# Gadersd/whisper-burn

Hardware: NVIDIA H100
Metric: audio-seconds/sec (higher is better)
Workload: dtype f32 (fp16-exact weights, fp32 activations/accumulate)

## Files before the change

### whisper-burn_b200/csrc/decoder4.cu

```cuda
#include <cooperative_groups.h>

#include "dec_common.cuh"

namespace cg = cooperative_groups;

namespace wb {

namespace {

#ifndef D4_ASYNC
#define D4_ASYNC 1
#endif
#define D4_EXCHANGE(IDX, RXBYTES, SEND, PF)                  \
    do {                                                     \
        WB_FINE();                                           \
        __syncthreads();                                     \
        WB_FINE();                                           \
        SEND();                                              \
        WB_FINE();                                           \
        if (D4_ASYNC) {                                      \
            PF();                                            \
            WB_FINE();                                       \
            xwait(xbar + (IDX), (RXBYTES), lc & 1u);         \
        } else {                                             \
            cluster_arrive();                                \
            PF();                                            \
            WB_FINE();                                       \
            cluster_wait();                                  \
        }                                                    \
    } while (0)
#ifndef D4_FINE
#define D4_FINE 0
#endif
#if D4_FINE
#define WB_FINE() WB_TRACE()
#else
#define WB_FINE() do { } while (0)
#endif

constexpr int CS = 16;
constexpr int LG_NBUF = 3;
constexpr int LG_RB = 8;
constexpr int KV_STG = 4;
#ifndef D4_L2_CKV_KEEP
#define D4_L2_CKV_KEEP 0
#endif
__device__ __forceinline__ uint64_t ckv_policy() { return D4_L2_CKV_KEEP ? l2_policy_evict_last() : l2_policy_evict_first(); }

__device__ __forceinline__ uint32_t smem_u32(const void* p) { return (uint32_t)__cvta_generic_to_shared(p); }
__device__ __forceinline__ void mbar_init(uint64_t* bar, uint32_t count) {
    asm volatile("mbarrier.init.shared::cta.b64 [%0], %1;" ::"r"(smem_u32(bar)), "r"(count));
}
__device__ __forceinline__ void mbar_expect_tx(uint64_t* bar, uint32_t bytes) {
    asm volatile("mbarrier.arrive.expect_tx.shared::cta.b64 _, [%0], %1;" ::"r"(smem_u32(bar)), "r"(bytes) : "memory");
}
__device__ __forceinline__ void mbar_wait(uint64_t* bar, uint32_t parity) {
    asm volatile(
        "{\n"
        ".reg .pred p;\n"
        "LG_WAIT:\n"
        "mbarrier.try_wait.parity.shared::cta.b64 p, [%0], %1;\n"
        "@p bra LG_DONE;\n"
        "bra LG_WAIT;\n"
        "LG_DONE:\n"
        "}\n" ::"r"(smem_u32(bar)),
        "r"(parity)
        : "memory");
}
__device__ __forceinline__ void cp_async16(void* dst, const void* src) {
    asm volatile("cp.async.cg.shared.global [%0], [%1], 16;" ::"r"(smem_u32(dst)), "l"(src) : "memory");
}
__device__ __forceinline__ void cp_async_wait_all() { asm volatile("cp.async.wait_all;" ::: "memory"); }

__device__ __forceinline__ void cluster_arrive() { asm volatile("barrier.cluster.arrive.release.aligned;" ::: "memory"); }
__device__ __forceinline__ void cluster_wait() { asm volatile("barrier.cluster.wait.acquire.aligned;" ::: "memory"); }

template <int NR, int VPL>
struct RowRegs {
    uint4 v[NR][VPL];
    float bias[NR];
    float bias_own;
};

template <int NR, int VPL>
__device__ __forceinline__ void load_rows(const __half* __restrict__ W, const float* __restrict__ bias, int K, int row0, int step,
                                          RowRegs<NR, VPL>& r, uint64_t pol) {
    const int lane = threadIdx.x & 31, nv = K / 8;
#pragma unroll
    for (int i = 0; i < NR; ++i) r.bias[i] = __ldg(bias + row0 + i * step);
    r.bias_own = __ldg(bias + row0 + min(lane >> 1, NR - 1) * step);
#pragma unroll
    for (int i = 0; i < NR; ++i) {
        const uint4* p = reinterpret_cast<const uint4*>(W + (int64_t)(row0 + i * step) * K);
#pragma unroll
        for (int j = 0; j < VPL; ++j) {
            const int v = j * 32 + lane;
            r.v[i][j] = v < nv ? ldg_l2(p + v, pol) : make_uint4(0, 0, 0, 0);
        }
    }
}
template <int NR>
__device__ __forceinline__ float warp_reduce_owner(const float (&acc)[NR]) {
    const int lane = threadIdx.x & 31;
    float v8[8], v4[4], v2[2];
    {
        const bool up = lane & 16;
#pragma unroll
        for (int i = 0; i < 8; ++i) {
            const float lo = i < NR ? acc[i] : 0.0f, hi = i + 8 < NR ? acc[i + 8] : 0.0f;
            const float recv = __shfl_xor_sync(0xffffffffu, up ? lo : hi, 16);
            v8[i] = (up ? hi : lo) + recv;
        }
    }
    {
        const bool up = lane & 8;
#pragma unroll
        for (int i = 0; i < 4; ++i) {
            const float recv = __shfl_xor_sync(0xffffffffu, up ? v8[i] : v8[i + 4], 8);
            v4[i] = (up ? v8[i + 4] : v8[i]) + recv;
        }
    }
    {
        const bool up = lane & 4;
#pragma unroll
        for (int i = 0; i < 2; ++i) {
            const float recv = __shfl_xor_sync(0xffffffffu, up ? v4[i] : v4[i + 2], 4);
            v2[i] = (up ? v4[i + 2] : v4[i]) + recv;
        }
    }
    const bool up = lane & 2;
    float v = (up ? v2[1] : v2[0]) + __shfl_xor_sync(0xffffffffu, up ? v2[0] : v2[1], 2);
    v += __shfl_xor_sync(0xffffffffu, v, 1);
    return v;
}

template <int NR, int VPL, bool REDUCE = true>
__device__ __forceinline__ void dot_rows1(const RowRegs<NR, VPL>& r, const float* xs, int K, float (&acc)[NR]) {
    const int lane = threadIdx.x & 31, nv = K / 8;
#pragma unroll
    for (int i = 0; i < NR; ++i) acc[i] = 0.0f;
#pragma unroll
    for (int j = 0; j < VPL; ++j) {
        const int v = j * 32 + lane;
        if (v < nv) {
            const float4 x0 = *reinterpret_cast<const float4*>(xs + v * 8);
            const float4 x1 = *reinterpret_cast<const float4*>(xs + v * 8 + 4);
#pragma unroll
            for (int i = 0; i < NR; ++i) {
                float w[8];
                cvt8(r.v[i][j], w);
                float a = acc[i];
                a = fmaf(w[0], x0.x, a); a = fmaf(w[1], x0.y, a); a = fmaf(w[2], x0.z, a); a = fmaf(w[3], x0.w, a);
                a = fmaf(w[4], x1.x, a); a = fmaf(w[5], x1.y, a); a = fmaf(w[6], x1.z, a); a = fmaf(w[7], x1.w, a);
                acc[i] = a;
            }
        }
    }
    if constexpr (REDUCE) {
#pragma unroll
        for (int i = 0; i < NR; ++i) acc[i] = warp_sum(acc[i]);
    }
}

__device__ __forceinline__ uint32_t mapa_u32(uint32_t addr, uint32_t rank) {
    uint32_t r;
    asm volatile("mapa.shared::cluster.u32 %0, %1, %2;" : "=r"(r) : "r"(addr), "r"(rank));
    return r;
}
__device__ __forceinline__ void st_async_v4(uint32_t raddr, const float4& v, uint32_t rbar) {
    asm volatile("st.async.shared::cluster.mbarrier::complete_tx::bytes.v4.f32 [%0], {%1, %2, %3, %4}, [%5];" ::"r"(raddr), "f"(v.x),
                 "f"(v.y), "f"(v.z), "f"(v.w), "r"(rbar)
                 : "memory");
}
__device__ __forceinline__ void put16(cg::cluster_group& cl, float* dst, uint64_t* bar, int dest, const float4& v) {
#if D4_ASYNC
    st_async_v4(mapa_u32(smem_u32(dst), (uint32_t)dest), v, mapa_u32(smem_u32(bar), (uint32_t)dest));
#else
    *reinterpret_cast<float4*>(cl.map_shared_rank(dst, dest)) = v;
#endif
}
template <int CNT>
__device__ __forceinline__ void put_slice(cg::cluster_group& cl, const float* stage_s, float* dst_local, uint64_t* bar) {
    static_assert(CNT % 4 == 0, "slice must be a whole number of 16-byte vectors");
    constexpr int Q = CNT / 4;
    for (int i = threadIdx.x; i < CS * Q; i += NT) {
        const int dest = i / Q, q = i - dest * Q;
        put16(cl, dst_local + 4 * q, bar, dest, reinterpret_cast<const float4*>(stage_s)[q]);
    }
}
__device__ __forceinline__ void xwait(uint64_t* bar, uint32_t bytes, uint32_t parity) {
    if (threadIdx.x == 0) mbar_expect_tx(bar, bytes);
    const uint32_t mb = smem_u32(bar);
    uint32_t done = 0;
    int spins = 0;
    while (!done) {
        asm volatile("{\n.reg .pred p;\nmbarrier.try_wait.parity.shared::cta.b64 p, [%1], %2;\nselp.u32 %0, 1, 0, p;\n}"
                     : "=r"(done)
                     : "r"(mb), "r"(parity)
                     : "memory");
        if (!done && ++spins > (1 << 24)) __trap();
    }
}

template <int PF>
struct XRegs {
    float4 v[PF];
};
__device__ __forceinline__ float4 add4(const float4& a, const float4& b) {
    return make_float4(__fadd_rn(a.x, b.x), __fadd_rn(a.y, b.y), __fadd_rn(a.z, b.z), __fadd_rn(a.w, b.w));
}
template <int PF>
__device__ __forceinline__ void x_update(XRegs<PF>& x, const float* src_s, const float* d_s, float* dst_s) {
    const int lane = threadIdx.x & 31;
#pragma unroll
    for (int k = 0; k < PF; ++k)
        x.v[k] = add4(reinterpret_cast<const float4*>(src_s)[lane + 32 * k], reinterpret_cast<const float4*>(d_s)[lane + 32 * k]);
    if (dst_s != nullptr && threadIdx.x < 32) {
#pragma unroll
        for (int k = 0; k < PF; ++k) reinterpret_cast<float4*>(dst_s)[lane + 32 * k] = x.v[k];
    }
}
template <int D, int PF>
__device__ __forceinline__ void ln_fetch(float* lnp, const float* __restrict__ g, const float* __restrict__ b, uint64_t pol) {
    const int lane = threadIdx.x & 31;
#pragma unroll
    for (int k = 0; k < PF; ++k) {
        cp_async16_l2(lnp + 4 * (lane + 32 * k), g + 4 * (lane + 32 * k), pol);
        cp_async16_l2(lnp + D + 4 * (lane + 32 * k), b + 4 * (lane + 32 * k), pol);
    }
}
template <int D, int PF>
__device__ __forceinline__ void ln_warp(XRegs<PF>& x, const float* gb_s, float eps, int eps_outside, float* out_s) {
    const int lane = threadIdx.x & 31;
    cp_async_wait_all();
    float s = 0.0f;
#pragma unroll
    for (int k = 0; k < PF; ++k) s += (x.v[k].x + x.v[k].y) + (x.v[k].z + x.v[k].w);
    s = warp_sum(s);
    const float mean = __fdiv_rn(s, (float)D);
    float q = 0.0f;
#pragma unroll
    for (int k = 0; k < PF; ++k) {
        x.v[k].x = __fsub_rn(x.v[k].x, mean); x.v[k].y = __fsub_rn(x.v[k].y, mean);
        x.v[k].z = __fsub_rn(x.v[k].z, mean); x.v[k].w = __fsub_rn(x.v[k].w, mean);
        q = fmaf(x.v[k].x, x.v[k].x, q); q = fmaf(x.v[k].y, x.v[k].y, q);
        q = fmaf(x.v[k].z, x.v[k].z, q); q = fmaf(x.v[k].w, x.v[k].w, q);
    }
    q = warp_sum(q);
    const float var = __fdiv_rn(q, (float)D);
    const float den = eps_outside ? __fadd_rn(__fsqrt_rn(var), eps) : __fsqrt_rn(__fadd_rn(var, eps));
    const float rinv = __fdiv_rn(1.0f, den);
#pragma unroll
    for (int k = 0; k < PF; ++k) {
        const float4 g = reinterpret_cast<const float4*>(gb_s)[lane + 32 * k];
        const float4 b = reinterpret_cast<const float4*>(gb_s + D)[lane + 32 * k];
        reinterpret_cast<float4*>(out_s)[lane + 32 * k] =
            make_float4(fmaf(__fmul_rn(x.v[k].x, rinv), g.x, b.x), fmaf(__fmul_rn(x.v[k].y, rinv), g.y, b.y),
                        fmaf(__fmul_rn(x.v[k].z, rinv), g.z, b.z), fmaf(__fmul_rn(x.v[k].w, rinv), g.w, b.w));
    }
    __syncwarp();
}

template <int D, int RC, typename KVT>
__global__ void __launch_bounds__(NT, 1)
dec4_kernel(const DecArgs a) {
    extern __shared__ __align__(16) float sm[];
    cg::cluster_group cl = cg::this_cluster();
    constexpr int H = D / 64;
    constexpr int VPL = (D / 8 + 31) / 32;
    constexpr int VPL4 = (4 * D / 8 + 31) / 32;
    constexpr int NR_QKV = 3 * D / (CS * NW), NR_D = D / (CS * NW), NR_H = 4 * D / (CS * NW);
    constexpr int KC = 2;
    const int L = a.L, V = a.V, R = a.R, t_max = a.t_max;
    const int tid = threadIdx.x, warp = tid >> 5, lane = tid & 31;
    const int rank = (int)cl.block_rank();
    const int row = blockIdx.x / CS;
    const bool active = row < R;

    float* lnp = sm + warp * 2 * D;
    float* qkv_s = sm + NW * 2 * D;
    float* att_s = qkv_s + 3 * D;
    float* dl_s = att_s + D;
    float* q2_s = dl_s + D;
    float* hid_s = q2_s + D;
    float* part_s = hid_s + 4 * D;
    float* wm = part_s + CS * 68;
    float* wl = wm + NW;
    float* wo = wl + NW;
    float* ao = wo + NW * 64;
    float* ML = ao + 64;
    constexpr int STG_N = 4 * D / CS > 68 ? 4 * D / CS : 68;
    float* stg_s = ML + 4;
    float* xb = stg_s + STG_N;
    float* xn_s = xb + 2 * D;
    float* red = xn_s + D;
    constexpr int RINGW = (LG_NBUF * LG_RB * D * 2 > KV_STG * 8 * 128 * 4) ? LG_NBUF * LG_RB * D * 2 : KV_STG * 8 * 128 * 4;
    constexpr int LG_PITCH = D * 2;
    uint8_t* ring = reinterpret_cast<uint8_t*>(red + NW * 4 * RC * 6);
    uint64_t* lg_bar = reinterpret_cast<uint64_t*>(ring + (size_t)NW * RINGW);
    uint64_t* kv_bar = lg_bar + NW * LG_NBUF;
    uint64_t* xbar = kv_bar + NW * KV_STG;
    uint4* pl_hi = reinterpret_cast<uint4*>(xbar + 8);
    uint4* pl_lo = pl_hi + (D / 32) * 32;
    if (lane == 0) {
        for (int j = 0; j < KV_STG; ++j) mbar_init(kv_bar + warp * KV_STG + j, 1);
        for (int j = 0; j < LG_NBUF; ++j) mbar_init(lg_bar + warp * LG_NBUF + j, 1);
        if (warp == 0)
            for (int j = 0; j < 8; ++j) mbar_init(xbar + j, 1);
        asm volatile("fence.mbarrier_init.release.cluster;" ::: "memory");
    }
    cl.sync();
    unsigned int lc = 0;
    unsigned int kv_count = 0;
    unsigned int lg_count = 0;
    unsigned int gen = 0;
    unsigned int lstep = 0;
    int tr_n = 0;
    const float scale = a.qk_scale;
    auto demote = [&]() {
        const size_t gt = (size_t)blockIdx.x * NT + tid, gn = (size_t)gridDim.x * NT;
        for (int l = 0; l < L; ++l) {
            const DecLayer& W = a.layers[l];
            l2_demote(W.Wqkv, (size_t)3 * D * D * 2, gt, gn);
            l2_demote(W.Wo, (size_t)D * D * 2, gt, gn);
            l2_demote(W.Wcq, (size_t)D * D * 2, gt, gn);
            l2_demote(W.Wco, (size_t)D * D * 2, gt, gn);
            l2_demote(W.W1, (size_t)4 * D * D * 2, gt, gn);
            l2_demote(W.W2, (size_t)4 * D * D * 2, gt, gn);
            l2_demote(W.ln1_g, D * 4, gt, gn); l2_demote(W.ln1_b, D * 4, gt, gn); l2_demote(W.ln2_g, D * 4, gt, gn);
            l2_demote(W.ln2_b, D * 4, gt, gn); l2_demote(W.ln3_g, D * 4, gt, gn); l2_demote(W.ln3_b, D * 4, gt, gn);
        }
        l2_demote(a.lnf_g, D * 4, gt, gn);
        l2_demote(a.lnf_b, D * 4, gt, gn);
        const size_t kv_bytes = (size_t)L * a.Rmax * t_max * D * sizeof(KVT);
        l2_demote(a.kc, kv_bytes, gt, gn);
        l2_demote(a.vc, kv_bytes, gt, gn);
        if (D4_L2_CKV_KEEP) l2_demote(a.ckv, (size_t)L * a.Mcap * 2 * D * sizeof(KVT), gt, gn);
    };
    WB_TRACE();

    const __half* nullw = nullptr;
    (void)nullw;
    for (int step = 0; step < a.n_steps; ++step) {
        const int p = a.pos0 + step;
        const bool want_logits = p >= a.logits_from;
        constexpr int KH = D / 2, NCH = KH / 32;
        constexpr uint32_t BLKB = 16 * KH * 2;
        static_assert(LG_NBUF * LG_RB * D * 2 >= LG_NBUF * (int)BLKB, "ring slot too small");
        const __half* Et = reinterpret_cast<const __half*>(a.E_tiled);
        const int v_tiles = (V + 15) / 16;
        const int t0w = (int)blockIdx.x + (int)gridDim.x * warp, tstep = (int)gridDim.x * NW;
        const int my_tiles = t0w < v_tiles ? (v_tiles - t0w + tstep - 1) / tstep : 0;
        const int total = my_tiles * 2;
        auto tile_of = [&](int i) { return t0w + i * tstep; };
        uint8_t* wring = ring + (size_t)warp * RINGW;
        uint64_t* wbar = lg_bar + warp * LG_NBUF;
        auto issue = [&](int it) {
            if (it < total && lane == 0) {
                const int vt = tile_of(it >> 1);
                const int slot = (int)((lg_count + (unsigned int)it) % LG_NBUF);
                mbar_expect_tx(wbar + slot, BLKB);
                bulk_g2s_l2(wring + (size_t)slot * BLKB, Et + ((int64_t)vt * 2 + (it & 1)) * 16 * KH, BLKB, wbar + slot, l2_policy_evict_first());
            }
        };
        uint4* gpl_hi = reinterpret_cast<uint4*>(a.att_pl);
        uint4* gpl_lo = gpl_hi + (D / 32) * 32;
        if (want_logits && !active) {
#pragma unroll
            for (int j = 0; j < LG_NBUF; ++j) issue(j);
        }
        if (active) {
            const int tok = __ldcg(a.tokens + (int64_t)row * t_max + p);
            const int xh = rank % H, xci = rank / H;
            const int xnch = (CS - xh + H - 1) / H;
            const int xw = __ldcg(a.row_window + row);
            const int xT = a.win_T[xw];
            const int64_t xoff = a.win_row_off[xw] * (int64_t)(2 * D) + (int64_t)xh * xT * 128;
            const int sub = lane >> 2, l4 = lane & 3;
            const bool self_fast = p + 1 <= NW * 16;
            constexpr int PF = D / 128;
            static_assert(D % 128 == 0, "row must be a whole number of float4s per lane");
            int xsel = 0;
            XRegs<PF> x;
#pragma unroll
            for (int k = 0; k < PF; ++k)
                x.v[k] = add4(__ldg(reinterpret_cast<const float4*>(a.tok_emb + (int64_t)tok * D) + lane + 32 * k),
                              __ldg(reinterpret_cast<const float4*>(a.pos_emb + (int64_t)p * D) + lane + 32 * k));
            if (warp == 0) {
#pragma unroll
                for (int k = 0; k < PF; ++k) reinterpret_cast<float4*>(xb)[lane + 32 * k] = x.v[k];
            }
            RowRegs<NR_QKV, VPL> w_qkv;
            load_rows<NR_QKV, VPL>(reinterpret_cast<const __half*>(a.layers[0].Wqkv), a.layers[0].bqkv, D, rank * (3 * D / CS) + warp, NW, w_qkv, l2_policy_evict_last());
            if (step == 0) ln_fetch<D, PF>(lnp, a.layers[0].ln1_g, a.layers[0].ln1_b, l2_policy_evict_last());
            __syncthreads();
            for (int l = 0; l < L; ++l) {
                const DecLayer& W = a.layers[l];
                KVT* kcl = reinterpret_cast<KVT*>(a.kc) + (size_t)l * a.Rmax * t_max * D;
                KVT* vcl = reinterpret_cast<KVT*>(a.vc) + (size_t)l * a.Rmax * t_max * D;
                if (l > 0) {
                    x_update<PF>(x, xb + xsel * D, dl_s, xb + (xsel ^ 1) * D);
                    xsel ^= 1;
                }
                ln_warp<D, PF>(x, lnp, W.ln1_eps, a.eps_outside, xn_s);
                ln_fetch<D, PF>(lnp, W.ln2_g, W.ln2_b, l2_policy_evict_last());
                {
                    float acc[NR_QKV];
                    dot_rows1<NR_QKV, VPL, false>(w_qkv, xn_s, D, acc);
                    float mine = warp_reduce_owner<NR_QKV>(acc);
                    mine = __fadd_rn(mine, w_qkv.bias_own);
                    const int j = warp + (lane >> 1) * NW;
                    if (rank * (3 * D / CS) + j < 2 * D) mine = __fmul_rn(mine, scale);
                    if (!(lane & 1) && (lane >> 1) < NR_QKV) stg_s[j] = mine;
                }
                RowRegs<NR_D, VPL> w_o;
                constexpr int SNV = sizeof(KVT) == 4 ? 4 : 2;
                uint8_t* sring = ring + (size_t)warp * RINGW;
                auto pre_s2 = [&]() {
                    load_rows<NR_D, VPL>(reinterpret_cast<const __half*>(W.Wo), W.bo, D, rank * (D / CS) + warp, NW, w_o, l2_policy_evict_last());
                    if (rank < H && self_fast) {
#pragma unroll
                        for (int u = 0; u < 2; ++u) {
                            const int j = warp + NW * (u * 8 + sub);
                            if (j < p) {
                                const int64_t o = ((int64_t)row * t_max + j) * D + rank * 64 + l4 * 16;
#pragma unroll
                                for (int c = 0; c < SNV; ++c) {
                                    cp_async16_l2(sring + ((u * 2 + 0) * 4 + c) * 512 + lane * 16, reinterpret_cast<const uint4*>(kcl + o) + c, l2_policy_evict_last());
                                    cp_async16_l2(sring + ((u * 2 + 1) * 4 + c) * 512 + lane * 16, reinterpret_cast<const uint4*>(vcl + o) + c, l2_policy_evict_last());
                                }
                            }
                        }
                    }
                };
                auto send_s1 = [&]() {
                    put_slice<3 * D / CS>(cl, stg_s, qkv_s + rank * (3 * D / CS), xbar + 0);
                    if (tid < 3 * D / CS) {
                        const int n = rank * (3 * D / CS) + tid;
                        const float v = stg_s[tid];
                        if (n >= 2 * D) vcl[((int64_t)row * t_max + p) * D + (n - 2 * D)] = (KVT)v;
                        else if (n >= D) kcl[((int64_t)row * t_max + p) * D + (n - D)] = (KVT)v;
                    }
                };
                D4_EXCHANGE(0, 3 * D * 4, send_s1, pre_s2);
                if (D4_ASYNC && !self_fast) cl.sync();
                WB_TRACE();
                if (rank < H) {
                    const int h = rank;
                    if (self_fast) {
                        cp_async_wait_all();
                        float q[16];
#pragma unroll
                        for (int c = 0; c < 4; ++c) {
                            const float4 t4 = *reinterpret_cast<const float4*>(qkv_s + h * 64 + l4 * 16 + c * 4);
                            q[c * 4] = t4.x; q[c * 4 + 1] = t4.y; q[c * 4 + 2] = t4.z; q[c * 4 + 3] = t4.w;
                        }
                        AttnAcc A;
                        A.m = -INFINITY;
                        A.l = 0.0f;
#pragma unroll
                        for (int c = 0; c < 16; ++c) A.o[c] = 0.0f;
#pragma unroll
                        for (int u = 0; u < 2; ++u) {
                            const int j = warp + NW * (u * 8 + sub);
                            float4 skk[4], svv[4];
                            if (j < p) {
                                if constexpr (sizeof(KVT) == 4) {
#pragma unroll
                                    for (int c = 0; c < 4; ++c) {
                                        skk[c] = *reinterpret_cast<const float4*>(sring + ((u * 2 + 0) * 4 + c) * 512 + lane * 16);
                                        svv[c] = *reinterpret_cast<const float4*>(sring + ((u * 2 + 1) * 4 + c) * 512 + lane * 16);
                                    }
                                } else {
#pragma unroll
                                    for (int c = 0; c < 2; ++c) {
                                        float w8[8];
                                        cvt8(*reinterpret_cast<const uint4*>(sring + ((u * 2 + 0) * 4 + c) * 512 + lane * 16), w8);
                                        skk[2 * c] = make_float4(w8[0], w8[1], w8[2], w8[3]); skk[2 * c + 1] = make_float4(w8[4], w8[5], w8[6], w8[7]);
                                        cvt8(*reinterpret_cast<const uint4*>(sring + ((u * 2 + 1) * 4 + c) * 512 + lane * 16), w8);
                                        svv[2 * c] = make_float4(w8[0], w8[1], w8[2], w8[3]); svv[2 * c + 1] = make_float4(w8[4], w8[5], w8[6], w8[7]);
                                    }
                                }
                            } else {
#pragma unroll
                                for (int c = 0; c < 4; ++c) { skk[c] = make_float4(0.f, 0.f, 0.f, 0.f); svv[c] = skk[c]; }
                            }
                            if (j == p) {
#pragma unroll
                                for (int c = 0; c < 4; ++c) {
                                    float4 k4 = *reinterpret_cast<const float4*>(qkv_s + D + h * 64 + l4 * 16 + c * 4);
                                    float4 v4 = *reinterpret_cast<const float4*>(qkv_s + 2 * D + h * 64 + l4 * 16 + c * 4);
                                    if constexpr (sizeof(KVT) == 2) {
                                        k4 = make_float4((float)(KVT)k4.x, (float)(KVT)k4.y, (float)(KVT)k4.z, (float)(KVT)k4.w);
                                        v4 = make_float4((float)(KVT)v4.x, (float)(KVT)v4.y, (float)(KVT)v4.z, (float)(KVT)v4.w);
                                    }
                                    skk[c] = k4;
                                    svv[c] = v4;
                                }
                            }
                            attn_regs_step(q, skk, svv, j <= p, A);
                        }
                        attn_merge_subs(A);
                        attn_cta_tail(A, wm, wl, wo, ao, ML);
                    } else {
                        const KVT* kb = kcl + h * 64;
                        const KVT* vb = vcl + h * 64;
                        auto kp = [&](int j) { return kb + ((int64_t)row * t_max + j) * D; };
                        auto vp = [&](int j) { return vb + ((int64_t)row * t_max + j) * D; };
                        attn_cta(qkv_s + h * 64, p + 1, kp, vp, wm, wl, wo, ao, ML);
                    }
                }
                auto send_s2 = [&]() {
                    if (rank < H) {
                        const int dest = tid >> 4, q = tid & 15;
                        const float4 o4 = reinterpret_cast<const float4*>(ao)[q];
                        const float den = ML[1];
                        put16(cl, att_s + rank * 64 + 4 * q, xbar + 1, dest,
                              make_float4(__fdiv_rn(o4.x, den), __fdiv_rn(o4.y, den), __fdiv_rn(o4.z, den), __fdiv_rn(o4.w, den)));
                    }
                };
                auto pf_none = [&]() {};
                D4_EXCHANGE(1, D * 4, send_s2, pf_none);
                WB_TRACE();
                {
                    float acc[NR_D];
                    dot_rows1<NR_D, VPL>(w_o, att_s, D, acc);
                    WB_FINE();
                    if (lane == 0) {
#pragma unroll
                        for (int i = 0; i < NR_D; ++i) stg_s[warp + i * NW] = __fadd_rn(acc[i], w_o.bias[i]);
                    }
                }
                RowRegs<NR_D, VPL> w_cq;
                auto pre_s4 = [&]() {
                    load_rows<NR_D, VPL>(reinterpret_cast<const __half*>(W.Wcq), W.bcq, D, rank * (D / CS) + warp, NW, w_cq, l2_policy_evict_last());
                    attn_bulk_prefill<KV_STG, KVT, true>(reinterpret_cast<const KVT*>(a.ckv) + (size_t)l * a.Mcap * 2 * D + xoff, xT, xci * NW + warp,
                                                         xnch * NW, ring + (size_t)warp * RINGW, kv_bar + warp * KV_STG, kv_count, ckv_policy());
                };
                auto send_s3 = [&]() { put_slice<D / CS>(cl, stg_s, dl_s + rank * (D / CS), xbar + 2); };
                D4_EXCHANGE(2, D * 4, send_s3, pre_s4);
                WB_TRACE();
                x_update<PF>(x, xb + xsel * D, dl_s, xb + (xsel ^ 1) * D);
                xsel ^= 1;
                ln_warp<D, PF>(x, lnp, W.ln2_eps, a.eps_outside, xn_s);
                ln_fetch<D, PF>(lnp, W.ln3_g, W.ln3_b, l2_policy_evict_last());
                WB_FINE();
                {
                    float acc[NR_D];
                    dot_rows1<NR_D, VPL>(w_cq, xn_s, D, acc);
                    WB_FINE();
                    if (lane == 0) {
#pragma unroll
                        for (int i = 0; i < NR_D; ++i) stg_s[warp + i * NW] = __fmul_rn(__fadd_rn(acc[i], w_cq.bias[i]), scale);
                    }
                }
                RowRegs<NR_D, VPL> w_co;
                auto pre_s6 = [&]() { load_rows<NR_D, VPL>(reinterpret_cast<const __half*>(W.Wco), W.bco, D, rank * (D / CS) + warp, NW, w_co, l2_policy_evict_last()); };
                auto send_s4 = [&]() { put_slice<D / CS>(cl, stg_s, q2_s + rank * (D / CS), xbar + 3); };
                D4_EXCHANGE(3, D * 4, send_s4, pre_s6);
                WB_TRACE();
                {
                    const int h = xh, ci = xci, nch = xnch, T = xT;
                    const KVT* kbase = reinterpret_cast<const KVT*>(a.ckv) + (size_t)l * a.Mcap * 2 * D + xoff;
                    AttnAcc A;
                    attn_warp_bulk<KV_STG, KVT, true>(q2_s + h * 64, kbase, T, ci * NW + warp, nch * NW, 0, ring + (size_t)warp * RINGW,
                                                      kv_bar + warp * KV_STG, kv_count, A, true, ckv_policy());
                    if (l == L - 1 && want_logits) {
                        __syncwarp();
                        asm volatile("fence.proxy.async.shared::cta;" ::: "memory");
#pragma unroll
                        for (int j = 0; j < LG_NBUF; ++j) issue(j);
                    }
                    if (lane < 4) {
#pragma unroll
                        for (int c = 0; c < 16; ++c) wo[warp * 64 + attn_bulk_dim<KVT>(lane, c)] = A.o[c];
                    }
                    if (lane == 0) { wm[warp] = A.m; wl[warp] = A.l; }
                    __syncthreads();
                    if (tid < 64) {
                        float M = -INFINITY;
#pragma unroll
                        for (int w2 = 0; w2 < NW; ++w2) M = fmaxf(M, wm[w2]);
                        float Ls = 0.0f, o = 0.0f;
#pragma unroll
                        for (int w2 = 0; w2 < NW; ++w2) {
                            const float m = wm[w2];
                            const float sc = m > -INFINITY ? expf(m - M) : 0.0f;
                            Ls += sc * wl[w2];
                            o += sc * wo[w2 * 64 + tid];
                        }
                        stg_s[4 + tid] = o;
                        if (tid < 4) stg_s[tid] = tid == 0 ? M : tid == 1 ? Ls : 0.0f;
                    }
                }
                auto send_s5 = [&]() { put_slice<68>(cl, stg_s, part_s + rank * 68, xbar + 4); };
                D4_EXCHANGE(4, CS * 68 * 4, send_s5, pf_none);
                WB_TRACE();
                for (int c = tid; c < D; c += NT) {
                    const int h = c / 64;
                    float M = -INFINITY;
                    for (int k = h; k < CS; k += H) M = fmaxf(M, part_s[k * 68]);
                    float den = 0.0f, num = 0.0f;
                    for (int k = h; k < CS; k += H) {
                        const float m = part_s[k * 68];
                        const float wgt = m > -INFINITY ? expf(m - M) : 0.0f;
                        den += wgt * part_s[k * 68 + 1];
                        num += wgt * part_s[k * 68 + 4 + (c & 63)];
                    }
                    att_s[c] = __fdiv_rn(num, den);
                }
                __syncthreads();
                {
                    float acc[NR_D];
                    dot_rows1<NR_D, VPL>(w_co, att_s, D, acc);
                    if (lane == 0) {
#pragma unroll
                        for (int i = 0; i < NR_D; ++i) stg_s[warp + i * NW] = __fadd_rn(acc[i], w_co.bias[i]);
                    }
                }
                RowRegs<NR_H, VPL> w_1;
                auto pre_s7 = [&]() { load_rows<NR_H, VPL>(reinterpret_cast<const __half*>(W.W1), W.b1, D, rank * (4 * D / CS) + warp, NW, w_1, l2_policy_evict_last()); };
                auto send_s6 = [&]() { put_slice<D / CS>(cl, stg_s, dl_s + rank * (D / CS), xbar + 5); };
                D4_EXCHANGE(5, D * 4, send_s6, pre_s7);
                WB_TRACE();
                x_update<PF>(x, xb + xsel * D, dl_s, xb + (xsel ^ 1) * D);
                xsel ^= 1;
                ln_warp<D, PF>(x, lnp, W.ln3_eps, a.eps_outside, xn_s);
                if (l == L - 1 && want_logits && rank == 0 && warp == 0) {
                    ln_fetch<D, PF>(lnp, a.lnf_g, a.lnf_b, l2_policy_evict_last());
                } else {
                    const DecLayer& Wn = a.layers[l + 1 < L ? l + 1 : 0];
                    ln_fetch<D, PF>(lnp, Wn.ln1_g, Wn.ln1_b, l2_policy_evict_last());
                }
                WB_FINE();
                {
                    float acc[NR_H];
                    dot_rows1<NR_H, VPL, false>(w_1, xn_s, D, acc);
                    float mine = warp_reduce_owner<NR_H>(acc);
                    mine = gelu_erf(__fadd_rn(mine, w_1.bias_own));
                    WB_FINE();
                    if (!(lane & 1) && (lane >> 1) < NR_H) stg_s[warp + (lane >> 1) * NW] = mine;
                }
                RowRegs<NR_D, VPL4> w_2;
                auto pre_s8 = [&]() { load_rows<NR_D, VPL4>(reinterpret_cast<const __half*>(W.W2), W.b2, 4 * D, rank * (D / CS) + warp, NW, w_2, l2_policy_evict_last()); };
                auto send_s7 = [&]() { put_slice<4 * D / CS>(cl, stg_s, hid_s + rank * (4 * D / CS), xbar + 6); };
                D4_EXCHANGE(6, 4 * D * 4, send_s7, pre_s8);
                WB_TRACE();
                {
                    float acc[NR_D];
                    dot_rows1<NR_D, VPL4>(w_2, hid_s, 4 * D, acc);
                    if (lane == 0) {
#pragma unroll
                        for (int i = 0; i < NR_D; ++i) stg_s[warp + i * NW] = __fadd_rn(acc[i], w_2.bias[i]);
                    }
                }
                auto pre_s1 = [&]() {
                    if (l + 1 < L)
                        load_rows<NR_QKV, VPL>(reinterpret_cast<const __half*>(a.layers[l + 1].Wqkv), a.layers[l + 1].bqkv, D, rank * (3 * D / CS) + warp, NW, w_qkv, l2_policy_evict_last());
                };
                auto send_s8 = [&]() { put_slice<D / CS>(cl, stg_s, dl_s + rank * (D / CS), xbar + 7); };
                D4_EXCHANGE(7, D * 4, send_s8, pre_s1);
                ++lc;
                WB_TRACE();
            }
            if (want_logits && rank == 0 && warp == 0) {
                x_update<PF>(x, xb + xsel * D, dl_s, nullptr);
                ln_warp<D, PF>(x, lnp, a.lnf_eps, a.eps_outside, xn_s);
#pragma unroll
                for (int k = 0; k < PF; ++k)
                    store_frag(gpl_hi, RC == 4 ? gpl_hi + 16 : gpl_lo, D / 32, row, 4 * (lane + 32 * k), reinterpret_cast<const float4*>(xn_s)[lane + 32 * k]);
                ln_fetch<D, PF>(lnp, a.layers[0].ln1_g, a.layers[0].ln1_b, l2_policy_evict_last());
            }
        }
        if (!want_logits) {
            if (D4_ASYNC && active) cl.sync();
            continue;
        }
        WB_TRACE();
        grid_sync(a.bar, gen);
        WB_TRACE();
        {
            const bool use_mask = a.is_special != nullptr && (a.mask_mode == 1 || (a.mask_mode == 2 && p + 1 <= 5));
            for (int i = tid; i < 2 * (D / 32) * 32; i += NT) cp_async16(pl_hi + i, gpl_hi + i);
            cp_async_wait_all();
            __syncthreads();
            WB_TRACE();
            const int g = lane >> 2, t = lane & 3;
            float m_run[2] = {-INFINITY, -INFINITY}, s_run[2] = {0.0f, 0.0f}, bv[2] = {-INFINITY, -INFINITY};
            int bi[2] = {INT_MAX, INT_MAX};
            float ah[4], al[4];
            unsigned int sp01 = 0;
#pragma unroll 1
            for (int it = 0; it < total; ++it) {
                const unsigned int cnt = lg_count + (unsigned int)it;
                const int slot = (int)(cnt % LG_NBUF);
                mbar_wait(wbar + slot, (cnt / LG_NBUF) & 1);
                const uint8_t* blk = wring + (size_t)slot * BLKB;
                const int half = it & 1;
                if (half == 0) {
#pragma unroll
                    for (int c = 0; c < 4; ++c) { ah[c] = 0.0f; al[c] = 0.0f; }
                    if (use_mask) {
                        const int n = tile_of(it >> 1) * 16 + g;
                        sp01 = (n < V ? ldg_l2(a.is_special + n, l2_policy_evict_first()) : 0u) | (n + 8 < V ? ldg_l2(a.is_special + n + 8, l2_policy_evict_first()) << 8 : 0u);
                    }
                }
#pragma unroll
                for (int c = 0; c < NCH; ++c) {
                    const uint4 a0 = *reinterpret_cast<const uint4*>(blk + (size_t)g * (KH * 2) + c * 64 + t * 16);
                    const uint4 a8 = *reinterpret_cast<const uint4*>(blk + (size_t)(g + 8) * (KH * 2) + c * 64 + t * 16);
                    const int chunk = half * NCH + c;
                    const uint4 bh = pl_hi[chunk * 32 + lane];
                    mma16816(ah, a0.x, a8.x, a0.y, a8.y, bh.x, bh.y);
                    mma16816(ah, a0.z, a8.z, a0.w, a8.w, bh.z, bh.w);
                    if constexpr (RC != 4) {
                        const uint4 bl = pl_lo[chunk * 32 + lane];
                        mma16816(al, a0.x, a8.x, a0.y, a8.y, bl.x, bl.y);
                        mma16816(al, a0.z, a8.z, a0.w, a8.w, bl.z, bl.w);
                    }
                }
                if (half == 1) {
                    const int n0 = tile_of(it >> 1) * 16;
#pragma unroll
                    for (int c = 0; c < 4; ++c) {
                        const int n = n0 + g + (c >> 1) * 8, e = c & 1;
                        if constexpr (RC == 4) al[c] = __shfl_xor_sync(0xffffffffu, ah[c], 2);
                        if (n < V && 2 * t + e < R) {
                            const float raw = fmaf(al[c], 1.0f / 2048.0f, ah[c]);
                            const float v = (use_mask && ((sp01 >> ((c >> 1) * 8)) & 0xffu)) ? __fadd_rn(raw, -INFINITY) : raw;
                            if (v > -INFINITY) {
                                if (v > m_run[e]) { s_run[e] = s_run[e] * expf(m_run[e] - v) + 1.0f; m_run[e] = v; }
                                else s_run[e] += expf(v - m_run[e]);
                            }
                            if (v > bv[e] || (v == bv[e] && n < bi[e])) { bv[e] = v; bi[e] = n; }
                        }
                    }
                }
                __syncwarp();
                issue(it + LG_NBUF);
            }
            lg_count += (unsigned int)total;
            WB_TRACE();
#pragma unroll
            for (int e = 0; e < 2; ++e) {
#pragma unroll
                for (int off = 4; off < 32; off <<= 1) {
                    const float m2 = __shfl_xor_sync(0xffffffffu, m_run[e], off), s2 = __shfl_xor_sync(0xffffffffu, s_run[e], off);
                    const float v2 = __shfl_xor_sync(0xffffffffu, bv[e], off);
                    const int i2 = __shfl_xor_sync(0xffffffffu, bi[e], off);
                    const float mn = fmaxf(m_run[e], m2);
                    s_run[e] = (m_run[e] > -INFINITY ? s_run[e] * expf(m_run[e] - mn) : 0.0f) + (m2 > -INFINITY ? s2 * expf(m2 - mn) : 0.0f);
                    m_run[e] = mn;
                    if (v2 > bv[e] || (v2 == bv[e] && i2 < bi[e])) { bv[e] = v2; bi[e] = i2; }
                }
                if (g == 0) {
                    float* rec = red + (warp * 8 + 2 * t + e) * 4;
                    rec[0] = m_run[e]; rec[1] = s_run[e]; rec[2] = bv[e]; rec[3] = __int_as_float(bi[e]);
                }
            }
            __syncthreads();
            if (tid < R) {
                float M = -INFINITY;
                for (int w2 = 0; w2 < NW; ++w2) M = fmaxf(M, red[(w2 * 8 + tid) * 4]);
                float Ssum = 0.0f, best_v = -INFINITY;
                int best_i = INT_MAX;
                for (int w2 = 0; w2 < NW; ++w2) {
                    const float* rec = red + (w2 * 8 + tid) * 4;
                    if (rec[0] > -INFINITY) Ssum += rec[1] * expf(rec[0] - M);
                    const int ci = __float_as_int(rec[3]);
                    if (rec[2] > best_v || (rec[2] == best_v && ci < best_i)) { best_v = rec[2]; best_i = ci; }
                }
                const int64_t o = (int64_t)blockIdx.x * R + tid;
                a.lg_m[o] = M;
                a.lg_s[o] = Ssum;
                a.lg_v[o * KC] = best_v;
                a.lg_i[o * KC] = best_i;
#pragma unroll
                for (int k = 1; k < KC; ++k) { a.lg_v[o * KC + k] = -INFINITY; a.lg_i[o * KC + k] = INT_MAX; }
            }
        }
        WB_TRACE();
        ++lstep;
        __syncthreads();
        if (tid == 0) {
            __threadfence();
            const unsigned int ticket = atomicAdd(a.bar + 1, 1u);
            reinterpret_cast<int*>(ML)[2] = (ticket == lstep * gridDim.x - 1) ? 1 : 0;
        }
        __syncthreads();
        WB_TRACE();
        if (reinterpret_cast<int*>(ML)[2]) {
            __threadfence();
            for (int r = warp; r < R; r += NW) {
                const int NP = gridDim.x;
                float rm[4], rs[4], rv[4];
                int ri[4];
#pragma unroll
                for (int k = 0; k < 4; ++k) {
                    const int c = min(lane + 32 * k, NP - 1);
                    rm[k] = __ldcg(a.lg_m + (int64_t)c * R + r);
                    rs[k] = __ldcg(a.lg_s + (int64_t)c * R + r);
                    rv[k] = __ldcg(a.lg_v + ((int64_t)c * R + r) * KC);
                    ri[k] = __ldcg(a.lg_i + ((int64_t)c * R + r) * KC);
                }
                float mx = -INFINITY;
#pragma unroll
                for (int k = 0; k < 4; ++k)
                    if (lane + 32 * k < NP) mx = fmaxf(mx, rm[k]);
#pragma unroll
                for (int o = 16; o > 0; o >>= 1) mx = fmaxf(mx, __shfl_xor_sync(0xffffffffu, mx, o));
                float se = 0.0f, bv = -INFINITY;
                int bi = INT_MAX;
#pragma unroll
                for (int k = 0; k < 4; ++k) {
                    if (lane + 32 * k < NP) {
                        if (rm[k] > -INFINITY) se += rs[k] * expf(rm[k] - mx);
                        if (ri[k] != INT_MAX && (rv[k] > bv || (rv[k] == bv && ri[k] < bi))) { bv = rv[k]; bi = ri[k]; }
                    }
                }
                se = warp_sum(se);
                const float lse = logf(se);
#pragma unroll
                for (int o = 16; o > 0; o >>= 1) {
                    const float ov = __shfl_xor_sync(0xffffffffu, bv, o);
                    const int oi = __shfl_xor_sync(0xffffffffu, bi, o);
                    if (ov > bv || (ov == bv && oi < bi)) { bv = ov; bi = oi; }
                }
                if (lane == 0) {
                    a.topk_id[r] = bi == INT_MAX ? -1 : bi;
                    a.topk_lp[r] = __fsub_rn(__fsub_rn(bv, mx), lse);
                    if (!__ldcg(a.finished + r)) {
                        a.tokens[(int64_t)r * t_max + p + 1] = bi;
                        a.lengths[r] = p + 2;
                        if (bi == a.eot) a.finished[r] = 1;
                    }
                }
            }
            __syncthreads();
            if (tid == 0) {
                __threadfence();
                asm volatile("st.release.gpu.global.u32 [%0], %1;" ::"l"(a.bar + 2), "r"(lstep) : "memory");
            }
        }
        WB_TRACE();
        if (tid == 0) {
            const long long t0 = clock64();
            while (ld_acquire(a.bar + 2) < lstep) {
                if (clock64() - t0 > 40000000000LL) __trap();
            }
        }
        __syncthreads();
        WB_TRACE();
        {
            int live = 0;
            for (int r = 0; r < R; ++r) live += __ldcg(a.finished + r) ? 0 : 1;
            if (live == 0) {
                if (blockIdx.x == 0 && tid == 0) { *a.pos = p + 1; *a.n_unfinished = 0; *a.steps_done = step + 1; }
                demote();
                return;
            }
        }
    }
    if (a.n_steps > 0 && a.pos0 + a.n_steps - 1 < a.logits_from) grid_sync(a.bar, gen);
    demote();
    if (blockIdx.x == 0 && tid == 0) {
        *a.pos = a.pos0 + a.n_steps;
        int live = 0;
        for (int r = 0; r < R; ++r) live += __ldcg(a.finished + r) ? 0 : 1;
        *a.n_unfinished = live;
        *a.steps_done = a.n_steps;
    }
}

template <int D, int RC>
size_t dec4_smem() {
    return sizeof(float) * ((size_t)(2 * NW + 13) * D + (4 * D / CS > 68 ? 4 * D / CS : 68) + CS * 68 + 2 * NW + NW * 64 + 64 + 4 + (size_t)NW * 4 * RC * 6 + 16) +
           (size_t)NW * std::max(LG_NBUF * LG_RB * D * 2, KV_STG * 8 * 128 * 4) + NW * LG_NBUF * 8 + NW * KV_STG * 8 + 8 * 8 + (size_t)2 * (D / 32) * 32 * 16 + 16;
}

template <int D, int RC, typename KVT>
bool launch4_t(const DecArgs& a, cudaStream_t st) {
    const void* k = (const void*)dec4_kernel<D, RC, KVT>;
    const size_t smem = dec4_smem<D, RC>();
    static ClusterLaunch cl;
    const int n_cl = std::min(cl.capacity(k, CS, NT, smem, "dec4"), 8);
    if (n_cl < 1 || a.R > n_cl) return false;
    void* args[] = {(void*)&a};
    cl.launch(k, CS, n_cl, NT, smem, args, st, "dec4");
    return true;
}

}

bool launch_dec4(const DecArgs& a, bool w_half, cudaStream_t st) {
    if (!w_half || a.R > 8 || a.R < 1 || a.k != 1 || !a.greedy || a.use_cur_tok || a.anc != nullptr || a.logits_out != nullptr) return false;
    if (a.H * 64 != a.d || a.H > CS || a.E_tiled == nullptr) return false;
#define WB_D4(DD)                                                                                         \
    do {                                                                                                  \
        if (a.kv_half) return a.R <= 4 ? launch4_t<DD, 4, __half>(a, st) : launch4_t<DD, 8, __half>(a, st); \
        return a.R <= 4 ? launch4_t<DD, 4, float>(a, st) : launch4_t<DD, 8, float>(a, st);                 \
    } while (0)
    if (a.d == 384) WB_D4(384);
    if (a.d == 128) WB_D4(128);
#undef WB_D4
    return false;
}

}
```

Before: 2506.

## Deepen vocab-projection prefetch ring and replace single-reducer argmax with redundant per-CTA reduction

Fixes shared memory at the maximum and gives non-row CTAs a deep ring of embedding tiles, with vocab tiles assigned as contiguous ranges weighted by each warp's ring depth. Idle CTAs start prefetching the next step's logits tiles right after arriving at the grid barrier. The last-arriver reduction plus its second release barrier becomes a single arrive/wait, after which every CTA does the top-1 reduction redundantly and keeps tokens and finished flags in shared memory. This removes one grid-wide serialization per step and global reads of tokens and finished flags, at the cost of duplicated reduction work and higher shared memory use, which may lower occupancy.

New measurement: 2540 (median of 6 runs). 1.01x the previous value.

```diff
diff --git a/whisper-burn_b200/csrc/decoder4.cu b/whisper-burn_b200/csrc/decoder4.cu
--- a/whisper-burn_b200/csrc/decoder4.cu
+++ b/whisper-burn_b200/csrc/decoder4.cu
@@ -42,6 +42,38 @@
 constexpr int LG_NBUF = 3;
 constexpr int LG_RB = 8;
 constexpr int KV_STG = 4;
+constexpr int DEC4_SMEM = 227 * 1024;
+
+template <int D, int RC>
+struct D4Smem {
+    static constexpr int STG_N = 4 * D / CS > 68 ? 4 * D / CS : 68;
+    static constexpr int STATE_F = (2 * NW + 13) * D + CS * 68 + 2 * NW + NW * 64 + 64 + 4 + STG_N;
+    static constexpr int RED_F = NW * 4 * RC * 6;
+    static constexpr int BLKB = 16 * (D / 2) * 2;
+    static constexpr int RINGW = (LG_NBUF * LG_RB * D * 2 > KV_STG * 8 * 128 * 4) ? LG_NBUF * LG_RB * D * 2 : KV_STG * 8 * 128 * 4;
+    static constexpr int NB_ROW = RINGW / BLKB;
+    static constexpr int NB_MAX = (DEC4_SMEM / BLKB + NW - 1) / NW;
+    static constexpr int TAIL_B = NW * NB_MAX * 8 + NW * KV_STG * 8 + 8 * 8 + 16 * 4 + 2 * (D / 32) * 32 * 16;
+    static constexpr int TAIL_OFF = DEC4_SMEM - TAIL_B;
+    static constexpr int S_DEEP = (TAIL_OFF - RED_F * 4) / BLKB;
+    static_assert(TAIL_OFF % 16 == 0 && (RED_F * 4) % 16 == 0, "bulk copy destinations and planes need 16-byte alignment");
+    static_assert(4 * (STATE_F + RED_F) + NW * RINGW <= TAIL_OFF, "the row CTA layout does not fit");
+    static_assert(NB_ROW >= 2 && NB_ROW <= NB_MAX && (S_DEEP + NW - 1) / NW <= NB_MAX, "ring slots");
+    static __host__ __device__ constexpr int deep_slot0(int w) { return w * (S_DEEP / NW) + (w < S_DEEP % NW ? w : S_DEEP % NW); }
+};
+
+template <int D, int RC>
+__host__ __device__ inline int vocab_first(int gw, int n_row_warps, int n_warps, int n_tiles) {
+    using SP = D4Smem<D, RC>;
+    auto held = [&](int g) -> int64_t {
+        if (g <= n_row_warps) return (int64_t)g * SP::NB_ROW;
+        const int h = g - n_row_warps;
+        return (int64_t)n_row_warps * SP::NB_ROW + (int64_t)(h / NW) * SP::S_DEEP + SP::deep_slot0(h % NW);
+    };
+    const int64_t all = held(n_warps), halves = 2 * (int64_t)n_tiles;
+    if (all >= halves) return (int)((int64_t)gw * n_tiles / n_warps);
+    return (int)((held(gw) * n_warps + (int64_t)gw * (halves - all)) / (2 * (int64_t)n_warps));
+}
 #ifndef D4_L2_CKV_KEEP
 #define D4_L2_CKV_KEEP 0
 #endif
@@ -289,26 +321,29 @@
     float* wo = wl + NW;
     float* ao = wo + NW * 64;
     float* ML = ao + 64;
-    constexpr int STG_N = 4 * D / CS > 68 ? 4 * D / CS : 68;
+    using SP = D4Smem<D, RC>;
+    constexpr int STG_N = SP::STG_N;
     float* stg_s = ML + 4;
     float* xb = stg_s + STG_N;
     float* xn_s = xb + 2 * D;
-    float* red = xn_s + D;
-    constexpr int RINGW = (LG_NBUF * LG_RB * D * 2 > KV_STG * 8 * 128 * 4) ? LG_NBUF * LG_RB * D * 2 : KV_STG * 8 * 128 * 4;
-    constexpr int LG_PITCH = D * 2;
-    uint8_t* ring = reinterpret_cast<uint8_t*>(red + NW * 4 * RC * 6);
-    uint64_t* lg_bar = reinterpret_cast<uint64_t*>(ring + (size_t)NW * RINGW);
-    uint64_t* kv_bar = lg_bar + NW * LG_NBUF;
+    float* red = active ? xn_s + D : sm;
+    constexpr int RINGW = SP::RINGW;
+    uint8_t* ring = reinterpret_cast<uint8_t*>(xn_s + D + SP::RED_F);
+    uint64_t* lg_bar = reinterpret_cast<uint64_t*>(reinterpret_cast<uint8_t*>(sm) + SP::TAIL_OFF);
+    uint64_t* kv_bar = lg_bar + NW * SP::NB_MAX;
     uint64_t* xbar = kv_bar + NW * KV_STG;
-    uint4* pl_hi = reinterpret_cast<uint4*>(xbar + 8);
+    int* tok_s = reinterpret_cast<int*>(xbar + 8);
+    int* fin_s = tok_s + 8;
+    uint4* pl_hi = reinterpret_cast<uint4*>(fin_s + 8);
     uint4* pl_lo = pl_hi + (D / 32) * 32;
     if (lane == 0) {
         for (int j = 0; j < KV_STG; ++j) mbar_init(kv_bar + warp * KV_STG + j, 1);
-        for (int j = 0; j < LG_NBUF; ++j) mbar_init(lg_bar + warp * LG_NBUF + j, 1);
+        for (int j = 0; j < SP::NB_MAX; ++j) mbar_init(lg_bar + warp * SP::NB_MAX + j, 1);
         if (warp == 0)
             for (int j = 0; j < 8; ++j) mbar_init(xbar + j, 1);
         asm volatile("fence.mbarrier_init.release.cluster;" ::: "memory");
     }
+    if (tid < R) fin_s[tid] = __ldcg(a.finished + tid);
     cl.sync();
     unsigned int lc = 0;
     unsigned int kv_count = 0;
@@ -339,38 +374,34 @@
     };
     WB_TRACE();
 
-    const __half* nullw = nullptr;
-    (void)nullw;
+    constexpr int KH = D / 2, NCH = KH / 32;
+    constexpr uint32_t BLKB = SP::BLKB;
+    const __half* Et = reinterpret_cast<const __half*>(a.E_tiled);
+    const int lg_nbuf = active ? SP::NB_ROW : SP::deep_slot0(warp + 1) - SP::deep_slot0(warp);
+    uint8_t* wring = active ? ring + (size_t)warp * RINGW : reinterpret_cast<uint8_t*>(sm + SP::RED_F) + (size_t)SP::deep_slot0(warp) * BLKB;
+    uint64_t* wbar = lg_bar + warp * SP::NB_MAX;
+    const int gw = (int)blockIdx.x * NW + warp, n_row_warps = R * CS * NW, n_warps = (int)gridDim.x * NW, v_tiles = (V + 15) / 16;
+    const int t0w = vocab_first<D, RC>(gw, n_row_warps, n_warps, v_tiles);
+    const int total = 2 * (vocab_first<D, RC>(gw + 1, n_row_warps, n_warps, v_tiles) - t0w);
+    auto issue = [&](int it) {
+        if (it < total && lane == 0) {
+            const unsigned int cnt = lg_count + (unsigned int)it;
+            const int slot = (int)(cnt % (unsigned int)lg_nbuf);
+            mbar_expect_tx(wbar + slot, BLKB);
+            bulk_g2s_l2(wring + (size_t)slot * BLKB, Et + ((int64_t)(t0w + (it >> 1)) * 2 + (it & 1)) * 16 * KH, BLKB, wbar + slot, l2_policy_evict_first());
+        }
+    };
+    uint4* gpl_hi = reinterpret_cast<uint4*>(a.att_pl);
+    uint4* gpl_lo = gpl_hi + (D / 32) * 32;
     for (int step = 0; step < a.n_steps; ++step) {
         const int p = a.pos0 + step;
         const bool want_logits = p >= a.logits_from;
-        constexpr int KH = D / 2, NCH = KH / 32;
-        constexpr uint32_t BLKB = 16 * KH * 2;
-        static_assert(LG_NBUF * LG_RB * D * 2 >= LG_NBUF * (int)BLKB, "ring slot too small");
-        const __half* Et = reinterpret_cast<const __half*>(a.E_tiled);
-        const int v_tiles = (V + 15) / 16;
-        const int t0w = (int)blockIdx.x + (int)gridDim.x * warp, tstep = (int)gridDim.x * NW;
-        const int my_tiles = t0w < v_tiles ? (v_tiles - t0w + tstep - 1) / tstep : 0;
-        const int total = my_tiles * 2;
-        auto tile_of = [&](int i) { return t0w + i * tstep; };
-        uint8_t* wring = ring + (size_t)warp * RINGW;
-        uint64_t* wbar = lg_bar + warp * LG_NBUF;
-        auto issue = [&](int it) {
-            if (it < total && lane == 0) {
-                const int vt = tile_of(it >> 1);
-                const int slot = (int)((lg_count + (unsigned int)it) % LG_NBUF);
-                mbar_expect_tx(wbar + slot, BLKB);
-                bulk_g2s_l2(wring + (size_t)slot * BLKB, Et + ((int64_t)vt * 2 + (it & 1)) * 16 * KH, BLKB, wbar + slot, l2_policy_evict_first());
-            }
-        };
-        uint4* gpl_hi = reinterpret_cast<uint4*>(a.att_pl);
-        uint4* gpl_lo = gpl_hi + (D / 32) * 32;
-        if (want_logits && !active) {
-#pragma unroll
-            for (int j = 0; j < LG_NBUF; ++j) issue(j);
+        const bool prev_logits = step > 0 && p - 1 >= a.logits_from;
+        if (want_logits && !active && !prev_logits) {
+            for (int j = 0; j < lg_nbuf; ++j) issue(j);
         }
         if (active) {
-            const int tok = __ldcg(a.tokens + (int64_t)row * t_max + p);
+            const int tok = prev_logits ? tok_s[row] : __ldcg(a.tokens + (int64_t)row * t_max + p);
             const int xh = rank % H, xci = rank / H;
             const int xnch = (CS - xh + H - 1) / H;
             const int xw = __ldcg(a.row_window + row);
@@ -569,7 +600,7 @@
                         __syncwarp();
                         asm volatile("fence.proxy.async.shared::cta;" ::: "memory");
 #pragma unroll
-                        for (int j = 0; j < LG_NBUF; ++j) issue(j);
+                        for (int j = 0; j < SP::NB_ROW; ++j) issue(j);
                     }
                     if (lane < 4) {
 #pragma unroll
@@ -693,15 +724,15 @@
 #pragma unroll 1
             for (int it = 0; it < total; ++it) {
                 const unsigned int cnt = lg_count + (unsigned int)it;
-                const int slot = (int)(cnt % LG_NBUF);
-                mbar_wait(wbar + slot, (cnt / LG_NBUF) & 1);
+                const int slot = (int)(cnt % (unsigned int)lg_nbuf);
+                mbar_wait(wbar + slot, (cnt / (unsigned int)lg_nbuf) & 1);
                 const uint8_t* blk = wring + (size_t)slot * BLKB;
                 const int half = it & 1;
                 if (half == 0) {
 #pragma unroll
                     for (int c = 0; c < 4; ++c) { ah[c] = 0.0f; al[c] = 0.0f; }
                     if (use_mask) {
-                        const int n = tile_of(it >> 1) * 16 + g;
+                        const int n = (t0w + (it >> 1)) * 16 + g;
                         sp01 = (n < V ? ldg_l2(a.is_special + n, l2_policy_evict_first()) : 0u) | (n + 8 < V ? ldg_l2(a.is_special + n + 8, l2_policy_evict_first()) << 8 : 0u);
                     }
                 }
@@ -720,7 +751,7 @@
                     }
                 }
                 if (half == 1) {
-                    const int n0 = tile_of(it >> 1) * 16;
+                    const int n0 = (t0w + (it >> 1)) * 16;
 #pragma unroll
                     for (int c = 0; c < 4; ++c) {
                         const int n = n0 + g + (c >> 1) * 8, e = c & 1;
@@ -737,7 +768,7 @@
                     }
                 }
                 __syncwarp();
-                issue(it + LG_NBUF);
+                issue(it + lg_nbuf);
             }
             lg_count += (unsigned int)total;
             WB_TRACE();
@@ -782,15 +813,24 @@
         WB_TRACE();
         ++lstep;
         __syncthreads();
+        if (tid == 0)
+            asm volatile("red.release.gpu.global.add.u32 [%0], 1;" ::"l"(a.bar + 1) : "memory");
+        const bool pf_next = !active && step + 1 < a.n_steps;
+        if (pf_next) {
+            __syncwarp();
+            asm volatile("fence.proxy.async.shared::cta;" ::: "memory");
+            for (int j = 0; j < lg_nbuf; ++j) issue(j);
+        }
+        WB_TRACE();
         if (tid == 0) {
-            __threadfence();
-            const unsigned int ticket = atomicAdd(a.bar + 1, 1u);
-            reinterpret_cast<int*>(ML)[2] = (ticket == lstep * gridDim.x - 1) ? 1 : 0;
+            const long long t0 = clock64();
+            while (ld_acquire(a.bar + 1) < lstep * gridDim.x) {
+                if (clock64() - t0 > 40000000000LL) __trap();
+            }
         }
         __syncthreads();
         WB_TRACE();
-        if (reinterpret_cast<int*>(ML)[2]) {
-            __threadfence();
+        {
             for (int r = warp; r < R; r += NW) {
                 const int NP = gridDim.x;
                 float rm[4], rs[4], rv[4];
@@ -827,35 +867,34 @@
                     if (ov > bv || (ov == bv && oi < bi)) { bv = ov; bi = oi; }
                 }
                 if (lane == 0) {
-                    a.topk_id[r] = bi == INT_MAX ? -1 : bi;
-                    a.topk_lp[r] = __fsub_rn(__fsub_rn(bv, mx), lse);
-                    if (!__ldcg(a.finished + r)) {
-                        a.tokens[(int64_t)r * t_max + p + 1] = bi;
-                        a.lengths[r] = p + 2;
-                        if (bi == a.eot) a.finished[r] = 1;
-                    }
+                    const bool was_finished = fin_s[r] != 0;
+                    if ((int)blockIdx.x == r * CS) {
+                        a.topk_id[r] = bi == INT_MAX ? -1 : bi;
+                        a.topk_lp[r] = __fsub_rn(__fsub_rn(bv, mx), lse);
+                        if (!was_finished) {
+                            a.tokens[(int64_t)r * t_max + p + 1] = bi;
+                            a.lengths[r] = p + 2;
+                            if (bi == a.eot) a.finished[r] = 1;
+                        }
+                    }
+                    tok_s[r] = !was_finished ? bi : step + 1 < a.n_steps ? __ldcg(a.tokens + (int64_t)r * t_max + p + 1) : 0;
+                    if (!was_finished && bi == a.eot) fin_s[r] = 1;
                 }
             }
             __syncthreads();
-            if (tid == 0) {
-                __threadfence();
-                asm volatile("st.release.gpu.global.u32 [%0], %1;" ::"l"(a.bar + 2), "r"(lstep) : "memory");
-            }
-        }
-        WB_TRACE();
-        if (tid == 0) {
-            const long long t0 = clock64();
-            while (ld_acquire(a.bar + 2) < lstep) {
-                if (clock64() - t0 > 40000000000LL) __trap();
-            }
-        }
-        __syncthreads();
+        }
         WB_TRACE();
         {
             int live = 0;
-            for (int r = 0; r < R; ++r) live += __ldcg(a.finished + r) ? 0 : 1;
+            for (int r = 0; r < R; ++r) live += fin_s[r] ? 0 : 1;
             if (live == 0) {
                 if (blockIdx.x == 0 && tid == 0) { *a.pos = p + 1; *a.n_unfinished = 0; *a.steps_done = step + 1; }
+                if (pf_next && lane == 0) {
+                    for (int j = 0; j < min(lg_nbuf, total); ++j) {
+                        const unsigned int cnt = lg_count + (unsigned int)j;
+                        mbar_wait(wbar + cnt % (unsigned int)lg_nbuf, (cnt / (unsigned int)lg_nbuf) & 1);
+                    }
+                }
                 demote();
                 return;
             }
@@ -866,22 +905,16 @@
     if (blockIdx.x == 0 && tid == 0) {
         *a.pos = a.pos0 + a.n_steps;
         int live = 0;
-        for (int r = 0; r < R; ++r) live += __ldcg(a.finished + r) ? 0 : 1;
+        for (int r = 0; r < R; ++r) live += fin_s[r] ? 0 : 1;
         *a.n_unfinished = live;
         *a.steps_done = a.n_steps;
     }
-}
-
-template <int D, int RC>
-size_t dec4_smem() {
-    return sizeof(float) * ((size_t)(2 * NW + 13) * D + (4 * D / CS > 68 ? 4 * D / CS : 68) + CS * 68 + 2 * NW + NW * 64 + 64 + 4 + (size_t)NW * 4 * RC * 6 + 16) +
-           (size_t)NW * std::max(LG_NBUF * LG_RB * D * 2, KV_STG * 8 * 128 * 4) + NW * LG_NBUF * 8 + NW * KV_STG * 8 + 8 * 8 + (size_t)2 * (D / 32) * 32 * 16 + 16;
 }
 
 template <int D, int RC, typename KVT>
 bool launch4_t(const DecArgs& a, cudaStream_t st) {
     const void* k = (const void*)dec4_kernel<D, RC, KVT>;
-    const size_t smem = dec4_smem<D, RC>();
+    const size_t smem = DEC4_SMEM;
     static ClusterLaunch cl;
     const int n_cl = std::min(cl.capacity(k, CS, NT, smem, "dec4"), 8);
     if (n_cl < 1 || a.R > n_cl) return false;
```
